# zyj0021200/simpleImageCaptionZoo

Measured on AMD Instinct MI355X. Metric: captions/sec (SCST step), BUTDDetection COCO14-size vocab, higher is better.
Workload: dtype f32

## Files before the change

### include/icz.h

```cpp
#ifndef ICZ_H_
#define ICZ_H_
#include <stddef.h>
#include <stdint.h>

#ifdef __cplusplus
extern "C" {
#endif

typedef enum {
    ICZ_OK = 0,
    ICZ_ERR_INVALID = -1,
    ICZ_ERR_HIP = -2,
    ICZ_ERR_STATE = -3,
    ICZ_ERR_NOMEM = -4
} icz_status;

const char* icz_last_error(void);
const char* icz_version(void);

typedef struct icz_butd icz_butd_t;

typedef struct {
    int32_t R;
    int32_t D;
// ... 268 lines not shown
                   const int32_t* img_ref_ptr, int32_t n_img, int32_t* stats_out, void* stream);
int icz_rouge_lcs(const int32_t* hyp_tok, const int32_t* hyp_ptr, const int32_t* ref_tok, const int32_t* ref_ptr,
                  const int32_t* img_ref_ptr, int32_t n_img, int32_t* lcs_out, void* stream);

int icz_gemm_f32(int32_t layout, const float* X, int32_t ldx, const float* W, int32_t ldw, const float* bias,
                 float* C, int32_t ldc, int32_t M, int32_t N, int32_t K, int32_t nsplit, float* workspace,
                 size_t workspace_floats, void* stream);
size_t icz_gemm_workspace_floats(int32_t M, int32_t N);
int icz_gemm_f32_seg(int32_t layout, int32_t nseg, const float* const* A, const int32_t* lda, const float* const* B, const int32_t* ldb,
                     const int32_t* K, const float* bias, float* C, int32_t ldc, int32_t M, int32_t N, int32_t nsplit, int32_t accumulate,
                     const int32_t* live, float* workspace, size_t workspace_floats, int32_t* nsplit_used, void* stream);
int icz_gemm_resident_pair(int32_t nseg_a, const float* const* A_a, const int32_t* lda_a, const float* const* B_a, const int32_t* ldb_a, const int32_t* K_a,
                           int32_t M_a, int32_t N_a, float* slabs_a, size_t slabs_a_floats, int32_t* nsplit_a,
                           int32_t nseg_b, const float* const* A_b, const int32_t* lda_b, const float* const* B_b, const int32_t* ldb_b, const int32_t* K_b,
                           int32_t M_b, int32_t N_b, float* slabs_b, size_t slabs_b_floats, int32_t* nsplit_b, const int32_t* live, void* stream);
int icz_gemm_set_big_cfg(int32_t cfg);
int icz_gemm_big_cfg_for(int32_t layout, int32_t M, int32_t N, int32_t K, int32_t nsplit);
int icz_gemm_tn_grouped(const float* dY, int32_t ldy, int32_t M, int32_t K, int32_t ngroups, const float* const* X, const int32_t* ldx,
                        const int32_t* cols, float* const* out, const int32_t* ldo, const int32_t* rows_live, void* stream);
int icz_gemm_tn_split_pick(int32_t M, int32_t N, int32_t K);
int icz_gemm_tn_split(const float* dY, int32_t ldy, int32_t M, const float* X, int32_t ldx, int32_t N, int32_t K, float* out, int32_t ldo,
                      float* workspace, size_t workspace_floats, const int32_t* rows_live, void* stream);
int icz_gemm_route_for(int32_t layout, int32_t M, int32_t N, int32_t nseg, const int32_t* K, int32_t nsplit);
int icz_gemm_split_for(int32_t layout, int32_t M, int32_t N, int32_t nseg, const int32_t* K, size_t workspace_floats);
int icz_gemm_tn_grouped_fits(int32_t M, int32_t K, int32_t ngroups, const int32_t* cols);
int icz_prof_begin(void);
int icz_prof_select(int32_t which);
int icz_prof_pair_overhead(void* stream, int32_t n, double* avg_us);
int icz_prof_end(double* avg_us, double* bytes_per_launch, double* flops_per_launch, long long* launches);
int icz_kprof_begin(void);
// ... 8 lines not shown
```

### simpleimagecaptionzoo_amd/_lib.py

```python
import ctypes as C
import os

_HERE = os.path.dirname(os.path.abspath(__file__))
LIB_PATH = os.path.join(_HERE, "libicz.so")


class IczError(RuntimeError):
    pass


GRAD_READY_CB = C.CFUNCTYPE(None, C.c_void_p, C.c_int32)


class ButdDims(C.Structure):
    _fields_ = [(n, C.c_int32) for n in ("R", "D", "H", "E", "A", "V", "max_rows", "max_len")]


BUTD_PARAM_FIELDS = (
    "embed_weight",
    "td_w_ih", "td_w_hh", "td_b_ih", "td_b_hh",
    "lm_w_ih", "lm_w_hh", "lm_b_ih", "lm_b_hh",
    "enc_att_v", "enc_att_g", "enc_att_b",
    "dec_att_v", "dec_att_g", "dec_att_b",
    "affine_v", "affine_g", "affine_b",
# ... 188 lines not shown
        "icz_ciderd_scores_csr": (C.c_int, [vp, vp, vp, i32, i32, vp, vp, vp, vp, vp, vp, vp, vp, vp, vp]),
        "icz_ngram_diversity": (C.c_int, [vp, vp, i32, i32, vp, vp]),
        "icz_bleu_stats": (C.c_int, [vp, vp, vp, vp, vp, i32, vp, vp]),
        "icz_rouge_lcs": (C.c_int, [vp, vp, vp, vp, vp, i32, vp, vp]),
        "icz_prof_begin": (C.c_int, []),
        "icz_prof_select": (C.c_int, [i32]),
        "icz_prof_pair_overhead": (C.c_int, [vp, i32, C.POINTER(C.c_double)]),
        "icz_prof_end": (C.c_int, [C.POINTER(C.c_double), C.POINTER(C.c_double), C.POINTER(C.c_double), C.POINTER(C.c_longlong)]),
        "icz_kprof_begin": (C.c_int, []),
        "icz_kprof_end": (C.c_int, [i32, C.POINTER(C.c_double), C.POINTER(C.c_longlong)]),
        "icz_prof_stream_rate": (C.c_int, [vp, C.c_size_t, i32, vp, C.POINTER(C.c_double)]),
        "icz_adam_clamp_multi": (C.c_int, [i32, C.POINTER(vp), C.POINTER(vp), C.POINTER(vp), C.POINTER(vp), C.POINTER(i64), f32, f32, i32, vp]),
        "icz_gemm_f32": (C.c_int, [i32, vp, i32, vp, i32, vp, vp, i32, i32, i32, i32, i32, vp, C.c_size_t, vp]),
        "icz_gemm_f32_seg": (C.c_int, [i32, i32, vp, vp, vp, vp, vp, vp, vp, i32, i32, i32, i32, i32, vp, vp, C.c_size_t, C.POINTER(i32), vp]),
        "icz_gemm_resident_pair": (C.c_int, [i32, vp, vp, vp, vp, vp, i32, i32, vp, C.c_size_t, C.POINTER(i32)] * 2 + [vp, vp]),
        "icz_gemm_workspace_floats": (C.c_size_t, [i32, i32]),
        "icz_gemm_set_big_cfg": (C.c_int, [i32]),
        "icz_gemm_big_cfg_for": (C.c_int, [i32, i32, i32, i32, i32]),
        "icz_gemm_tn_grouped": (C.c_int, [vp, i32, i32, i32, i32, vp, vp, vp, vp, vp, vp, vp]),
        "icz_gemm_tn_split_pick": (C.c_int, [i32, i32, i32]),
        "icz_gemm_tn_split": (C.c_int, [vp, i32, i32, vp, i32, i32, i32, vp, i32, vp, C.c_size_t, vp, vp]),
        "icz_gemm_route_for": (C.c_int, [i32, i32, i32, i32, vp, i32]),
        "icz_gemm_split_for": (C.c_int, [i32, i32, i32, i32, vp, C.c_size_t]),
        "icz_gemm_tn_grouped_fits": (C.c_int, [i32, i32, i32, vp]),
    }
    for name, (res, args) in sig.items():
        try:
            fn = getattr(L, name)
        except AttributeError as e:
            raise IczError("libicz.so lacks symbol %s (stale build?)" % name) from e
# ... 18 lines not shown
```

### simpleimagecaptionzoo_amd/butd.py

```python
import ctypes as C

import torch

from . import _lib
from ._lib import BUTD_PARAM_KEYS, ButdDims, ButdParams, Rng, check, lib, ptr, stream_ptr
from .handle import GraphDecoderHandle


def make_rng(seed=0, uniforms=None, emb_mask=None, att_mask=None, out_mask=None):
    r = Rng()
    r.seed = int(seed) & 0xFFFFFFFFFFFFFFFF
    keep = []
    for name, t, dt in (("uniforms", uniforms, torch.float32), ("emb_mask", emb_mask, torch.uint8),
                        ("att_mask", att_mask, torch.uint8), ("out_mask", out_mask, torch.uint8)):
        if t is not None:
            if t.dtype != dt or not t.is_cuda or not t.is_contiguous():
                raise _lib.IczError("%s must be a contiguous %s CUDA tensor" % (name, dt))
            setattr(r, name, t.data_ptr())
            keep.append(t)
    r._keep = keep
    return r


class ButdHandle(GraphDecoderHandle):
# ... 121 lines not shown
        M, N = (int(out.shape[0]), int(out.shape[1])) if out is not None else (1, 1)
    dev = out.device if out is not None else (As[0].device if n else "cuda")
    if out is None and not raw_slabs:
        out = torch.empty(M, N, device=dev, dtype=torch.float32)
    if workspace is None:
        workspace = torch.empty(max(lib().icz_gemm_workspace_floats(M, N), max(nsplit, 1) * M * N), device=dev, dtype=torch.float32)
    used = C.c_int32(0)
    c = None if raw_slabs else out
    check(lib().icz_gemm_f32_seg(code, n, ap, lda, bp, ldb, kk, ptr(bias), ptr(c), c.stride(0) if c is not None else N, M, N, int(nsplit),
                                 1 if accumulate else 0, ptr(live), ptr(workspace), workspace.numel(), C.byref(used), stream_ptr()))
    if info is not None:
        info["nsplit"] = used.value
    return workspace[:used.value * M * N].view(used.value, M, N) if raw_slabs else out


def gemm_resident_pair(As_a, Bs_a, As_b, Bs_b, slabs_a=None, slabs_b=None, live=None):
    ta, tb = _seg_tables("nt", As_a, Bs_a), _seg_tables("nt", As_b, Bs_b)
    bufs = []
    for (n, _, _, _, _, kk, M, N), buf, As in ((ta, slabs_a, As_a), (tb, slabs_b, As_b)):
        if M is None:
            raise _lib.IczError("gemm_resident_pair: a problem without segments")
        if buf is None:
            buf = torch.empty(max(sum(kk) // 256, 1) * M * N, device=As[0].device, dtype=torch.float32)
        bufs.append(buf)
    na, nb = C.c_int32(0), C.c_int32(0)
    args = []
    for (n, ap, lda, bp, ldb, kk, M, N), buf, used in ((ta, bufs[0], na), (tb, bufs[1], nb)):
        args += [n, ap, lda, bp, ldb, kk, M, N, ptr(buf), buf.numel(), C.byref(used)]
    check(lib().icz_gemm_resident_pair(*args, ptr(live), stream_ptr()))
    return tuple(buf[:u.value * t[6] * t[7]].view(u.value, t[6], t[7]) for t, buf, u in ((ta, bufs[0], na), (tb, bufs[1], nb)))


def gemm_set_big_cfg(cfg):
    check(lib().icz_gemm_set_big_cfg(int(cfg)))


def gemm_tn_grouped(dY, Xs, outs=None, rows_live=None):
    K, M = dY.shape
    n = len(Xs)
    if outs is None:
        outs = [torch.empty(M, x.shape[1], device=dY.device, dtype=torch.float32) for x in Xs]
    xp = (C.c_void_p * n)(*[x.data_ptr() for x in Xs])
    op = (C.c_void_p * n)(*[o.data_ptr() for o in outs])
    ldx = (C.c_int32 * n)(*[x.stride(0) for x in Xs])
# ... 44 lines not shown
```

### simpleimagecaptionzoo_amd/csrc/butd.hip

```cpp
#include <vector>

#include "butd_impl.h"

namespace icz {

int Butd::init(const icz_butd_dims& d) {
    dims = d;
    ICZ_REQUIRE(d.R > 0 && d.R <= 64, "butd: R=%d must be in 1..64 (36 boxes / 49 grid cells)", d.R);
    ICZ_REQUIRE(d.D % 4 == 0 && d.H % 4 == 0 && d.E % 4 == 0 && d.A % 4 == 0, "butd: D,H,E,A must be multiples of 4");
    ICZ_REQUIRE(d.V > 3 && d.max_rows > 0 && d.max_len > 0, "butd: bad V/max_rows/max_len");
    const size_t rows = d.max_rows, H = d.H, D = d.D, E = d.E, A = d.A, V = d.V, R = d.R;
    ICZ_TRY(alloc((void**)&w_enc, sizeof(float) * A * D));
    ICZ_TRY(alloc((void**)&w_dec, sizeof(float) * A * H));
    ICZ_TRY(alloc((void**)&w_aff, sizeof(float) * A));
    const size_t Vp = pad_vocab(d.V);
    ICZ_TRY(alloc((void**)&w_pred, sizeof(float) * Vp * H));
    ICZ_TRY(alloc((void**)&n_enc, sizeof(float) * A));
    ICZ_TRY(alloc((void**)&n_dec, sizeof(float) * A));
    ICZ_TRY(alloc((void**)&n_aff, sizeof(float) * 4));
    ICZ_TRY(alloc((void**)&n_pred, sizeof(float) * V));
    ICZ_TRY(alloc((void**)&mean, sizeof(float) * rows * D));
    ICZ_TRY(alloc((void**)&premean, sizeof(float) * rows * 4 * H));
    ICZ_TRY(alloc((void**)&enc_ctx, sizeof(float) * rows * R * A));
    for (int i = 0; i < 2; ++i) {
// ... 13 lines not shown
    ICZ_TRY(alloc((void**)&it, sizeof(int64_t) * rows));
    ICZ_TRY(alloc_scalars(mem));
    size_t nmax = 4 * H;
    if (A > nmax) nmax = A;
    if (V > nmax) nmax = V;
    ws_floats = (size_t)TARGET_WGS * 4096 * 2 + rows * nmax;
    {
        const size_t kmax = 2 * H + (E > D ? E : D), r128 = rows < 128 ? rows : 128;
        const size_t need = (kmax / 256 + 1) * r128 * 4 * H;
        if (need > ws_floats) ws_floats = need;
    }
    ICZ_TRY(alloc((void**)&ws, sizeof(float) * ws_floats));
    ICZ_TRY(mem.synced());
    if (const char* e = getenv("ICZ_EARLY_OUT")) early_out = atoi(e) != 0;
    if (const char* e = getenv("ICZ_MERGE_SMALL")) { const int n = atoi(e); if (n >= 0 && n <= 32) merge_small = n; }
    return ICZ_OK;
}

int Butd::refresh(hipStream_t st) {
    ICZ_REQUIRE(bound, "butd: parameters not bound");
    const int A = dims.A, D = dims.D, H = dims.H, V = dims.V;
    WeightNormTable wt = {};
    int nb = 0;
    auto add = [&](const float* v, const float* g, float* w, float* norm, int rows, int cols) {
        wt.j[wt.count++] = {v, g, w, norm, rows, cols, nb};
        nb += cdiv(rows, 4);
    };
    add(P.enc_att_v, P.enc_att_g, w_enc, n_enc, A, D);
    add(P.dec_att_v, P.dec_att_g, w_dec, n_dec, A, H);
    add(P.affine_v, P.affine_g, w_aff, n_aff, 1, A);
// ... 214 lines not shown
    }
    b->P = *p;
    b->bound = true;
    b->fresh = false;
    return ICZ_OK;
}

int icz_butd_set_option(icz_butd_t* h, const char* name, int32_t value) {
    ICZ_REQUIRE(h && name, "icz_butd_set_option: null argument");
    Butd* b = reinterpret_cast<Butd*>(h);
    if (strcmp(name, "graphs") == 0) { b->use_graphs = value != 0; return ICZ_OK; }
    if (strcmp(name, "concurrent") == 0) { b->concurrent = value != 0; return ICZ_OK; }
    if (strcmp(name, "early_out") == 0) { b->early_out = value != 0; return ICZ_OK; }
    if (strcmp(name, "small_nt") == 0) { b->small_nt = value != 0; return ICZ_OK; }
    if (strcmp(name, "group_att") == 0) { b->group_att = value != 0; return ICZ_OK; }
    if (strcmp(name, "merge_small") == 0) {
        ICZ_REQUIRE(value >= 0 && value <= 32, "icz_butd_set_option: merge_small %d outside 0..32", value);
        b->merge_small = value;
        return ICZ_OK;
    }
    set_error("icz_butd_set_option: unknown option '%s'", name);
    return ICZ_ERR_INVALID;
}

int icz_butd_set_mask_sum_global(icz_butd_t* h, const float* mask_sum_global_dev, void* stream) {
    return set_norm_global("icz_butd_set_mask_sum_global", reinterpret_cast<Butd*>(h), mask_sum_global_dev, stream);
}

int icz_butd_set_grad_callback(icz_butd_t* h, icz_grad_ready_cb cb, void* user) {
    ICZ_REQUIRE(h, "null handle");
// ... 39 lines not shown
```

### simpleimagecaptionzoo_amd/csrc/butd_impl.h

```cpp
#pragma once
#include <vector>
#include <stdint.h>

#include "decoder_core.h"

namespace icz {

struct StepIO {
    int rows;
    const float* feats;
    const int32_t* img_of_row;
    int rows_per_img;
    const int64_t* it;
    bool emb_ready;
    const float *h1_in, *c1_in, *h2_in, *c2_in;
    float *h1_out, *c1_out, *h2_out, *c2_out;
    float* emb_out;
    float* gates_td_out;
    float* gates_lm_out;
    float* dec_ctx_out;
    float* alpha_out;
    float* alpha_out2; int alpha2_stride;
    float* ctx_out;
    float* h2drop_out;
// ... 48 lines not shown
    int refresh_transposes(hipStream_t st);

    int alloc(void** p, size_t bytes) { return mem.alloc(p, bytes); }
    int init(const icz_butd_dims& d);
    int refresh(hipStream_t st);
    int gemm_nt(GemmArgs& g, const float* bias, hipStream_t st);
    int prologue(const float* feats, int n_img, hipStream_t st);
    int step(const StepIO& s, hipStream_t st);
    int zero_state(int rows, int which, hipStream_t st);
    int greedy(const float* feats, int B, int max_len, int64_t* ids_out, float* alphas_out, hipStream_t st);

    GraphCache gc{24};
    bool use_graphs = false;
    bool concurrent = true;
    uintptr_t opt_bits() const {
        return (concurrent ? 1 : 0) + (early_out ? 2 : 0) + 4 * merge_small + (small_nt ? 256 : 0) + (group_att ? 512 : 0);
    }
    int greedy_impl(const float* feats, int B, int max_len, int64_t* ids_out, float* alphas_out, hipStream_t st);
    int sample_impl(const float* feats, int B, int T, int64_t* seq_out, float* logp_out, hipStream_t st);
    int greedy_chain(const float* feats, int B, int max_len, int64_t* ids_out, float* alphas_out, hipStream_t st, bool scst = false);
    int sample_chain(const float* feats, int B, int T, int64_t* seq_out, float* logp_out, hipStream_t st, int row0 = 0, int64_t* ids_out = nullptr);
    int rollouts(const float* feats, int B, int T, const icz_rng* r, int64_t* ids_out, int64_t* seq_out, float* logp_out, hipStream_t st);
    int rollouts_impl(const float* feats, int B, int T, int64_t* ids_out, int64_t* seq_out, float* logp_out, hipStream_t st);
    SideStream side;
    SideStream low;
    icz_grad_ready_cb grad_cb = nullptr; void* grad_cb_user = nullptr;
    int sample_backward_impl(const float* reward, const icz_butd_params& G, float* loss_out, float* mask_sum_out, hipStream_t st,
                             int phases = 0xF, bool fire_cb = true);
    bool bptt_joined = false;
    int merge_small = 8;
    int cur_rows = 0, cur_row0 = 0;
    bool early_out = true;
    bool bptt_early_out = false;
    bool small_nt = true;
    int cur_K = 1, cur_nimg = 0;
    bool group_att = false;

    const float* seam_feats = nullptr;
    int vocab() const override { return dims.V; }
    int row_capacity() const override { return dims.max_rows; }
    bool refreshed() const override { return fresh; }
    bool compact_step() const override { return true; }
    EmbSlot emb_slot() const override { return {P.embed_weight, emb, dims.E, 1}; }
    DeviceBuffers& buffers() override { return mem; }
    int prologue(const float* feats, int n_img, int k, const int32_t* img_of_row, hipStream_t st) override;
    int step(int rows, const int64_t* it, const int32_t* img_of_row, int rows_per_img, int cur, bool slabs, LogitsView* out,
             hipStream_t st) override;
    void gather(const int32_t* src_row, int rows, int fan, hipStream_t st) override;

// ... 26 lines not shown
```

### simpleimagecaptionzoo_amd/csrc/butd_train.hip

```cpp
#include <math.h>

#include "butd_impl.h"

namespace icz {

__global__ void sample_init_kernel(uint8_t* unf, int* nunf, int64_t* tok, int B, int T) {
    const int i = blockIdx.x * blockDim.x + threadIdx.x;
    if (i < B) { unf[i] = 1; tok[i] = 1; }
    if (i < T) nunf[i] = 0;
}

int Butd::ensure_train(int B, int T) {
    if (tb.B >= B && tb.T >= T) return ICZ_OK;
    ICZ_REQUIRE(B <= 2 * dims.max_rows, "butd: batch %d exceeds capacity %d", B, dims.max_rows);
    ICZ_REQUIRE(T <= XE_MAX_T, "butd: %d steps exceed the limit of %d", T, XE_MAX_T);
    if (tb.B > B) B = tb.B;
    if (tb.T > T) T = tb.T;
    if (dims.max_len > T) T = dims.max_len;
    if (!mem.training.empty()) {
        ICZ_TRY(mem.release_training(&gc));
        tb = TrainBuf();
        drop_loss_buffers();
    }
    if (!wt_lm_ih && wt_possible()) {
// ... 446 lines not shown
        }
        const bool rdg = wt_lm_ih && wt_fresh && bt > 32 && bt <= 64 && gemm_slab_floats(bt, D + H, 4 * H / 256) <= tb.xfloats &&
                         gemm_slab_floats(bt, H, 2 * (4 * H / 256)) <= tb.xfloats;
        const bool tdg = small_nt && wt_lm_ih && wt_fresh && bt <= 32;
        const GemmLayout lay = (rdg || tdg) ? GEMM_NT : GEMM_NN;
        const float* const dglm = tb.dGlm + slot * 4 * H;
        const float* const dgtd = tb.dGtd + slot * 4 * H;
        auto wseg = [&](const float* dg, const float* w_t, const float* w, int ldw) -> GemmSeg {
            return lay == GEMM_NT ? GemmSeg{dg, w_t, 4 * H, 4 * H, 4 * H} : GemmSeg{dg, w, 4 * H, ldw, 4 * H};
        };
        auto dgrad = [&](GemmArgs g, float* slab, int* ns) -> int {
            if (!rdg) return gemm_auto(lay, g, slab, tb.xfloats, ns, st);
            *ns = gemm_resident_x3_nsplit(g);
            return gemm_slabs(GEMM_NT, g, *ns, slab, tb.xfloats, st, "butd");
        };
        ICZ_TRY(dgrad(gemm_args({wseg(dglm, wt_lm_ih, P.lm_w_ih, D + H)}, bt, D + H, tb.X[0], D + H, live), tb.X[0], &ns1));
        {
            const int dparts = cdiv(D, DALPHA_COLS);
            hipLaunchKernelGGL(att_bwd_dalpha_kernel, dim3(bt, dparts), dim3(256), 0, st, tb.X[0], ns1, D + H, bt, feats, R, D, tb.dalpha, live, imgk);
            AttBwdDdecArgs da = {enc_ctx, tb.dec + slot * A, w_aff, tb.alpha + slot * R, tb.dalpha, tb.dDec + slot * A, tb.dS + slot * R, R, A, dparts, live, imgk};
            hipLaunchKernelGGL(att_bwd_ddec_kernel, dim3(bt, cdiv(A, 256)), dim3(256), 0, st, da, d_att);
            GemmArgs g = gemm_args({{tb.dDec + slot * A, w_dec, A, H, A}}, bt, H, tb.X[1], H, live);
            ICZ_TRY(gemm_auto(GEMM_NN, g, tb.X[1], tb.xfloats, &ns2, st));
        }
        {
            LstmBwdArgs a = {};
            a.dh_a = bnext ? tb.X[3] : nullptr; a.ns_a = ns4; a.lda_a = H; a.rows_a = bnext;
            a.dh_b = tb.X[0] + D; a.ns_b = ns1; a.lda_b = D + H; a.rows_b = bt;
            a.dh_c = tb.X[1]; a.ns_c = ns2; a.lda_c = H; a.rows_c = bt;
            a.dc_in = bnext ? tb.dc1[cur] : nullptr; a.dc_in_rows = bnext;
            a.gates = tb.gtd + slot * 4 * H;
            a.c_prev = tb.c1 + slot * H; a.c_cur = tb.c1 + slot * H + sH;
            a.dgates = tb.dGtd + slot * 4 * H; a.dc_prev = tb.dc1[cur ^ 1];
            a.rows = bt; a.H = H; a.live = live; a.carry_live = carry_live;
            hipLaunchKernelGGL(lstm_bwd_point_kernel, dim3(cdiv(H, 256), bt), dim3(256), 0, st, a, d_off);
        }
        if (t > 0) {
            const GemmArgs g3 = gemm_args({wseg(dglm, wt_lm_hh, P.lm_w_hh, H), wseg(dgtd, wt_td_ih_h2, P.td_w_ih, H + D + E)}, bt, H, tb.X[2], H, live);
            const GemmArgs g4 = gemm_args({wseg(dgtd, wt_td_hh, P.td_w_hh, H)}, bt, H, tb.X[3], H, live);
            if (rdg) {
                ns3 = gemm_resident_x3_nsplit(g3); ns4 = gemm_resident_x3_nsplit(g4);
                ICZ_REQUIRE(gemm_slab_floats(bt, H, ns3) <= tb.xfloats, "butd: slab buffer too small for the dgrad slabs");
                ICZ_TRY(gemm_resident_x3_pair(g3, g4, st));
            } else {
                ICZ_TRY(dgrad(g3, tb.X[2], &ns3));
                ICZ_TRY(dgrad(g4, tb.X[3], &ns4));
            }
        }
        bnext = bt;
        cur ^= 1;
    }
    return ICZ_OK;
    };
    const int s_loop = loop();
    if (grad_cb || s_loop != ICZ_OK) {
// ... 214 lines not shown
```

### simpleimagecaptionzoo_amd/csrc/gemm_f32.h

```cpp
#pragma once
#include "icz_common.h"

namespace icz {

constexpr int GEMM_MAX_SEG = 4;
constexpr int GEMM_BM = 64, GEMM_BN = 64, GEMM_BK = 64;

enum GemmLayout { GEMM_NT = 0, GEMM_NN = 1, GEMM_TN = 2 };

struct GemmSeg {
    const float* A;
    const float* B;
    int lda, ldb;
    int K;
    const int64_t* gather;
};

struct GemmArgs {
    GemmSeg seg[GEMM_MAX_SEG];
    int nseg;
    int M, N;
    float* out;
    int ldo;
    const float* bias;
// ... 2 lines not shown
    int accumulate;
    int spread;
    const int* live;
    const int* rows_live;
};

int gemm_f32(GemmLayout layout, const GemmArgs& a, hipStream_t stream);
int gemm_route(GemmLayout layout, const GemmArgs& a);
int gemm_pick_split(const GemmArgs& a, int target_wgs, GemmLayout layout = GEMM_NT);
int gemm_pick_split_balanced(const GemmArgs& a, GemmLayout layout, size_t slab_capacity_floats);
size_t gemm_slab_floats(int M, int N, int nsplit);
int gemm_normalize_split(GemmLayout layout, const GemmArgs& a, int nsplit);
int gemm_fit_split(GemmLayout layout, const GemmArgs& a, int nsplit, size_t capacity_floats);

bool gemm_resident_x3_fits(const GemmArgs& a);
int gemm_resident_x3_stages(const GemmArgs& a);
int gemm_resident_x3_nsplit(const GemmArgs& a);
int gemm_resident_x3(const GemmArgs& a, hipStream_t stream);
bool gemm_resident_x3_pair_fits(const GemmArgs& a, const GemmArgs& b);
int gemm_resident_x3_pair(const GemmArgs& a, const GemmArgs& b, hipStream_t stream);
int gemm_predict(const float* x, int H, const float* w_pred, const float* bias, int rows, int V, int Vp, float* logits, int ldl,
                 float* ws, size_t ws_cap_floats, int* pred_nsplit, hipStream_t st, const int* live = nullptr);

int gemm_big_x3(GemmLayout layout, const GemmArgs& a, int cfg, hipStream_t stream);
int gemm_big_cfg(GemmLayout layout, const GemmArgs& a);
int gemm_big_switch();
void gemm_set_big_cfg(int cfg);
constexpr int GEMM_MAX_COLGROUPS = 4;
struct GemmColGroup { const float* B; int ldb; int cols; float* out; int ldo; };
bool gemm_tn_grouped_fits(int M, int K, const GemmColGroup* groups, int ngroups);
int gemm_tn_grouped(const float* dY, int ldy, int M, int K, const GemmColGroup* groups, int ngroups, const int* rows_live, hipStream_t stream);

int gemm_tn_split_pick(int M, int N, int K);
int gemm_tn_split(const float* dY, int ldy, int M, const float* X, int ldx, int N, int K, int nsplit, float* slabs, const int* rows_live, hipStream_t st);
struct GemmSwitches { bool tn_x3, nn_x3, nt_x3big, resident_x3, resident_m128, predict_slabs, resident_k512; unsigned prof_every; int big_cfg; };
// ... 4 lines not shown
```

### simpleimagecaptionzoo_amd/csrc/gemm_f32.hip

```cpp
#include <stdlib.h>

#include <array>
#include <mutex>
#include <set>
#include <vector>

#include "gemm_ops.h"

namespace icz {

static int total_chunks(const GemmArgs& a, int bk = GEMM_BK) {
    int t = 0;
    for (int s = 0; s < a.nseg; ++s) t += cdiv(a.seg[s].K, bk);
    return t;
}

template <int BK>
struct ChunkCursorT {
    int seg, k0;
    const float* A; const float* B;
    int lda, ldb, K;
    __device__ __forceinline__ void load_seg(const GemmArgs& a) {
        const GemmSeg& g = a.seg[seg];
        A = g.A; B = g.B; lda = g.lda; ldb = g.ldb; K = g.K;
// ... 1259 lines not shown
    if (C) {
        g.out = C; g.ldo = ldc;
        ICZ_TRY(gemm_finished(lay, g, ns, bias, workspace, workspace_floats, st, "icz_gemm_f32_seg"));
    } else {
        g.out = workspace; g.ldo = N; g.bias = bias; g.nsplit = ns;
        ICZ_TRY(gemm_f32(lay, g, st));
    }
    if (nsplit_used) *nsplit_used = ns;
    return ICZ_OK;
}

int icz_gemm_resident_pair(int32_t nseg_a, const float* const* A_a, const int32_t* lda_a, const float* const* B_a, const int32_t* ldb_a, const int32_t* K_a,
                           int32_t M_a, int32_t N_a, float* slabs_a, size_t slabs_a_floats, int32_t* nsplit_a,
                           int32_t nseg_b, const float* const* A_b, const int32_t* lda_b, const float* const* B_b, const int32_t* ldb_b, const int32_t* K_b,
                           int32_t M_b, int32_t N_b, float* slabs_b, size_t slabs_b_floats, int32_t* nsplit_b, const int32_t* live, void* stream) {
    GemmArgs ga, gb;
    ICZ_TRY(seg_args("icz_gemm_resident_pair (first)", nseg_a, A_a, lda_a, B_a, ldb_a, K_a, M_a, N_a, &ga));
    ICZ_TRY(seg_args("icz_gemm_resident_pair (second)", nseg_b, A_b, lda_b, B_b, ldb_b, K_b, M_b, N_b, &gb));
    ga.out = slabs_a; ga.ldo = N_a; ga.live = live;
    gb.out = slabs_b; gb.ldo = N_b; gb.live = live;
    ICZ_REQUIRE(gemm_resident_x3_pair_fits(ga, gb), "icz_gemm_resident_pair: the two problems do not share a stage form of the resident kernel");
    ga.nsplit = gemm_resident_x3_nsplit(ga);
    gb.nsplit = gemm_resident_x3_nsplit(gb);
    ICZ_REQUIRE(ga.nsplit > 1 && gb.nsplit > 1, "icz_gemm_resident_pair: slab products only (one k range: %d, %d)", ga.nsplit, gb.nsplit);
    ICZ_TRY(check_args(GEMM_NT, ga));
    ICZ_TRY(check_args(GEMM_NT, gb));
    ICZ_REQUIRE(((uintptr_t)slabs_a & 15) == 0 && ((uintptr_t)slabs_b & 15) == 0, "icz_gemm_resident_pair: slabs must be 16-byte aligned");
    ICZ_REQUIRE(gemm_slab_floats(M_a, N_a, ga.nsplit) <= slabs_a_floats && gemm_slab_floats(M_b, N_b, gb.nsplit) <= slabs_b_floats,
                "icz_gemm_resident_pair: slab buffers too small (%d x %d x %d, %d x %d x %d)", ga.nsplit, M_a, N_a, gb.nsplit, M_b, N_b);
    ICZ_TRY(gemm_resident_x3_pair(ga, gb, (hipStream_t)stream));
    if (nsplit_a) *nsplit_a = ga.nsplit;
    if (nsplit_b) *nsplit_b = gb.nsplit;
    return ICZ_OK;
}

int icz_gemm_set_big_cfg(int32_t cfg) {
    ICZ_REQUIRE(cfg >= -2 && cfg <= 5, "icz_gemm_set_big_cfg: %d", cfg);
    gemm_set_big_cfg(cfg);
    return ICZ_OK;
}

int icz_gemm_big_cfg_for(int32_t layout, int32_t M, int32_t N, int32_t K, int32_t nsplit) {
    if (layout < 0 || layout > 2 || M <= 0 || N <= 0 || K <= 0) return -1;
    GemmArgs g = {};
    g.nseg = 1;
// ... 64 lines not shown
```

### simpleimagecaptionzoo_amd/csrc/gemm_resident_x3.hip

```cpp
#include <stdlib.h>

#include <type_traits>

#include "gemm_f32.h"

namespace icz {

template <int I, int N, class F>
__device__ __forceinline__ void sk_static_for(F&& f) {
    if constexpr (I < N) {
        f(std::integral_constant<int, I>{});
        sk_static_for<I + 1, N>(f);
    }
}

typedef __attribute__((ext_vector_type(8))) __bf16 sk_bf16x8;
typedef __attribute__((ext_vector_type(4))) uint32_t sk_u32x4;
typedef __attribute__((ext_vector_type(2))) uint32_t sk_u32x2;

__device__ __forceinline__ uint32_t sk_cvt_pk_bf16(float lo, float hi) {
    uint32_t r;
    asm("v_cvt_pk_bf16_f32 %0, %1, %2" : "=v"(r) : "v"(lo), "v"(hi));
    return r;
}
// ... 489 lines not shown
    });
    stamp(31);
}

template <int D, bool STAMPS = false>
__global__ __launch_bounds__(256) void gemm_resident_x3_m128_kernel(GemmArgs a) {
    resident_x3_m128_body<D, STAMPS>(a, blockIdx.x);
}
constexpr size_t rs_m128_lds_bytes() { return (size_t)3 * 128 * rs_pb(2) * 2; }

static int rs_total_stages(const GemmArgs& a) {
    int tot = 0;
    for (int s = 0; s < a.nseg; ++s) tot += a.seg[s].K / SK_BK;
    return tot;
}
int gemm_resident_x3_stages(const GemmArgs& a) {
    const int tot = rs_total_stages(a);
    if (gemm_switches().resident_k512 && a.M <= 64 && tot % 8 == 0) return 8;
    return tot % 4 == 0 ? 4 : 0;
}
static bool rs_shape_ok(const GemmArgs& a) {
    if (!gemm_switches().resident_x3 || a.M <= 32 || a.M > (gemm_switches().resident_m128 ? 128 : 64) || a.N % 4 || a.accumulate) return false;
    for (int s = 0; s < a.nseg; ++s)
        if (a.seg[s].K % SK_BK || a.seg[s].gather) return false;
    return rs_total_stages(a) >= 8 && gemm_resident_x3_stages(a) > 0;
}
bool gemm_resident_x3_fits(const GemmArgs& a) { return a.N >= 2048 && rs_shape_ok(a); }
int gemm_resident_x3_nsplit(const GemmArgs& a) { return rs_total_stages(a) / gemm_resident_x3_stages(a); }

template <int NSR, bool STAMPS>
static int rs_launch(const GemmArgs& a, hipStream_t stream) {
    constexpr size_t lds = rs_lds_bytes<4, NSR>();
    static bool attr = false;
    if (!attr) {
        ICZ_CHECK_HIP(hipFuncSetAttribute(reinterpret_cast<const void*>(gemm_resident_x3_kernel<4, NSR, 2, 3, STAMPS>), hipFuncAttributeMaxDynamicSharedMemorySize, (int)lds));
        attr = true;
    }
    hipLaunchKernelGGL((gemm_resident_x3_kernel<4, NSR, 2, 3, STAMPS>), dim3(cdiv(a.N, 256) * a.nsplit), dim3(256), lds, stream, a);
    ICZ_CHECK_HIP(hipGetLastError());
    return ICZ_OK;
}

#ifndef RS_K512_D
// ... 34 lines not shown
    GemmArgs a = a_in;
    const int nsr = gemm_resident_x3_stages(a);
    ICZ_REQUIRE(rs_shape_ok(a) && a.nsplit == gemm_resident_x3_nsplit(a) && a.chunks_per_split == nsr,
                "gemm_resident_x3: launch does not match the kernel's fixed decomposition (nsplit %d)", a.nsplit);
    ICZ_REQUIRE(a.nsplit > 1 || a.ldo >= a.N, "gemm_resident_x3: output row stride %d below N = %d", a.ldo, a.N);
#ifdef ICZ_DEV
    if (rs_dev_env("ICZ_DEV_STAMPS")) {
        if (!g_sk_stamps) ICZ_CHECK_HIP(hipMalloc((void**)&g_sk_stamps, sizeof(unsigned long long) * 32 * 4096));
        a.bias = reinterpret_cast<const float*>(g_sk_stamps);
        return a.M > 64 ? rs_launch_m128<true>(a, stream) : (nsr == 8 ? rs_launch_k512<true>(a, stream) : rs_launch<4, true>(a, stream));
    }
#endif
    return a.M > 64 ? rs_launch_m128<false>(a, stream) : (nsr == 8 ? rs_launch_k512<false>(a, stream) : rs_launch<4, false>(a, stream));
}

bool gemm_resident_x3_pair_fits(const GemmArgs& a, const GemmArgs& b) {
    return a.M <= 64 && b.M <= 64 && rs_shape_ok(a) && rs_shape_ok(b) && gemm_resident_x3_stages(a) == gemm_resident_x3_stages(b) && a.N >= 512 && b.N >= 512;
}
int gemm_resident_x3_pair(const GemmArgs& a_in, const GemmArgs& b_in, hipStream_t stream) {
    ICZ_REQUIRE(gemm_resident_x3_pair_fits(a_in, b_in), "gemm_resident_x3_pair: shapes outside the kernel's decomposition");
    GemmPair g;
    g.a = a_in; g.b = b_in;
    const int nsr = gemm_resident_x3_stages(g.a), tilew = nsr == 8 ? 128 : 256;
    for (GemmArgs* p : {&g.a, &g.b}) {
        p->nsplit = gemm_resident_x3_nsplit(*p);
        p->chunks_per_split = nsr;
        p->bias = nullptr;
        ICZ_REQUIRE(p->out && p->nsplit > 1, "gemm_resident_x3_pair: slab output expected");
    }
    g.first = cdiv(g.a.N, tilew) * g.a.nsplit;
    constexpr size_t lds = rs_lds_bytes<4, 4>();
    static bool attr = false;
    if (!attr) {
        ICZ_CHECK_HIP(hipFuncSetAttribute(reinterpret_cast<const void*>(gemm_resident_x3_pair_kernel<4, 4, 2, 3>), hipFuncAttributeMaxDynamicSharedMemorySize, (int)lds));
        ICZ_CHECK_HIP(hipFuncSetAttribute(reinterpret_cast<const void*>(gemm_resident_x3_pair_kernel<4, 8, 1, RS_K512_D, 4>), hipFuncAttributeMaxDynamicSharedMemorySize, (int)lds));
        attr = true;
    }
    const dim3 grid(g.first + cdiv(g.b.N, tilew) * g.b.nsplit);
    if (nsr == 8) hipLaunchKernelGGL((gemm_resident_x3_pair_kernel<4, 8, 1, RS_K512_D, 4>), grid, dim3(256), lds, stream, g);
    else hipLaunchKernelGGL((gemm_resident_x3_pair_kernel<4, 4, 2, 3>), grid, dim3(256), lds, stream, g);
    ICZ_CHECK_HIP(hipGetLastError());
    return ICZ_OK;
}

int gemm_predict(const float* x, int H, const float* w_pred, const float* bias, int rows, int V, int Vp, float* logits, int ldl,
                 float* ws, size_t ws_cap_floats, int* pred_nsplit, hipStream_t st, const int* live) {
    GemmArgs g = {};
    g.nseg = 1;
    g.live = live;
    g.seg[0] = {x, w_pred, H, H, H, nullptr};
    g.M = rows; g.N = Vp; g.out = ws; g.ldo = Vp;
    if (gemm_switches().predict_slabs && pred_nsplit && ws && gemm_resident_x3_fits(g) && gemm_resident_x3_nsplit(g) > 1 &&
        gemm_slab_floats(rows, Vp, gemm_resident_x3_nsplit(g)) <= ws_cap_floats) {
        g.nsplit = gemm_resident_x3_nsplit(g);
// ... 18 lines not shown
```

Baseline: 11870.

## Regroup BPTT dgrad GEMMs by producer into paired resident launches

In the backward-through-time step, the dgrad GEMMs are regrouped by producer. The lm_ih dgrad is paired with the lm_hh part of the former fused g3, and the td_ih part is paired with td_hh in a second paired launch. This lets the lm-derived products start earlier and balances the work across the two launches. It also adds a 4-stage, 128-wide tile variant of the paired resident kernel, selectable by stage count and made the default via dgrad_by_producer=2, which raises the split count and grid size for small M. The cost is more slab partials to reduce and a new kernel instantiation, and the path only runs when the slab buffers fit.

```diff
diff --git a/include/icz.h b/include/icz.h
--- a/include/icz.h
+++ b/include/icz.h
@@ -306,6 +306,11 @@
                            int32_t M_a, int32_t N_a, float* slabs_a, size_t slabs_a_floats, int32_t* nsplit_a,
                            int32_t nseg_b, const float* const* A_b, const int32_t* lda_b, const float* const* B_b, const int32_t* ldb_b, const int32_t* K_b,
                            int32_t M_b, int32_t N_b, float* slabs_b, size_t slabs_b_floats, int32_t* nsplit_b, const int32_t* live, void* stream);
+int icz_gemm_resident_pair_stages(int32_t nseg_a, const float* const* A_a, const int32_t* lda_a, const float* const* B_a, const int32_t* ldb_a, const int32_t* K_a,
+                                  int32_t M_a, int32_t N_a, float* slabs_a, size_t slabs_a_floats, int32_t* nsplit_a,
+                                  int32_t nseg_b, const float* const* A_b, const int32_t* lda_b, const float* const* B_b, const int32_t* ldb_b, const int32_t* K_b,
+                                  int32_t M_b, int32_t N_b, float* slabs_b, size_t slabs_b_floats, int32_t* nsplit_b, int32_t stages,
+                                  const int32_t* live, void* stream);
 int icz_gemm_set_big_cfg(int32_t cfg);
 int icz_gemm_big_cfg_for(int32_t layout, int32_t M, int32_t N, int32_t K, int32_t nsplit);
 int icz_gemm_tn_grouped(const float* dY, int32_t ldy, int32_t M, int32_t K, int32_t ngroups, const float* const* X, const int32_t* ldx,
diff --git a/simpleimagecaptionzoo_amd/_lib.py b/simpleimagecaptionzoo_amd/_lib.py
--- a/simpleimagecaptionzoo_amd/_lib.py
+++ b/simpleimagecaptionzoo_amd/_lib.py
@@ -226,6 +226,7 @@
         "icz_gemm_f32": (C.c_int, [i32, vp, i32, vp, i32, vp, vp, i32, i32, i32, i32, i32, vp, C.c_size_t, vp]),
         "icz_gemm_f32_seg": (C.c_int, [i32, i32, vp, vp, vp, vp, vp, vp, vp, i32, i32, i32, i32, i32, vp, vp, C.c_size_t, C.POINTER(i32), vp]),
         "icz_gemm_resident_pair": (C.c_int, [i32, vp, vp, vp, vp, vp, i32, i32, vp, C.c_size_t, C.POINTER(i32)] * 2 + [vp, vp]),
+        "icz_gemm_resident_pair_stages": (C.c_int, [i32, vp, vp, vp, vp, vp, i32, i32, vp, C.c_size_t, C.POINTER(i32)] * 2 + [i32, vp, vp]),
         "icz_gemm_workspace_floats": (C.c_size_t, [i32, i32]),
         "icz_gemm_set_big_cfg": (C.c_int, [i32]),
         "icz_gemm_big_cfg_for": (C.c_int, [i32, i32, i32, i32, i32]),
diff --git a/simpleimagecaptionzoo_amd/butd.py b/simpleimagecaptionzoo_amd/butd.py
--- a/simpleimagecaptionzoo_amd/butd.py
+++ b/simpleimagecaptionzoo_amd/butd.py
@@ -159,7 +159,7 @@
     return workspace[:used.value * M * N].view(used.value, M, N) if raw_slabs else out
 
 
-def gemm_resident_pair(As_a, Bs_a, As_b, Bs_b, slabs_a=None, slabs_b=None, live=None):
+def gemm_resident_pair(As_a, Bs_a, As_b, Bs_b, slabs_a=None, slabs_b=None, live=None, stages=0):
     ta, tb = _seg_tables("nt", As_a, Bs_a), _seg_tables("nt", As_b, Bs_b)
     bufs = []
     for (n, _, _, _, _, kk, M, N), buf, As in ((ta, slabs_a, As_a), (tb, slabs_b, As_b)):
@@ -172,7 +172,10 @@
     args = []
     for (n, ap, lda, bp, ldb, kk, M, N), buf, used in ((ta, bufs[0], na), (tb, bufs[1], nb)):
         args += [n, ap, lda, bp, ldb, kk, M, N, ptr(buf), buf.numel(), C.byref(used)]
-    check(lib().icz_gemm_resident_pair(*args, ptr(live), stream_ptr()))
+    if stages:
+        check(lib().icz_gemm_resident_pair_stages(*args, int(stages), ptr(live), stream_ptr()))
+    else:
+        check(lib().icz_gemm_resident_pair(*args, ptr(live), stream_ptr()))
     return tuple(buf[:u.value * t[6] * t[7]].view(u.value, t[6], t[7]) for t, buf, u in ((ta, bufs[0], na), (tb, bufs[1], nb)))
 
 
diff --git a/simpleimagecaptionzoo_amd/csrc/butd.hip b/simpleimagecaptionzoo_amd/csrc/butd.hip
--- a/simpleimagecaptionzoo_amd/csrc/butd.hip
+++ b/simpleimagecaptionzoo_amd/csrc/butd.hip
@@ -51,6 +51,7 @@
     ICZ_TRY(mem.synced());
     if (const char* e = getenv("ICZ_EARLY_OUT")) early_out = atoi(e) != 0;
     if (const char* e = getenv("ICZ_MERGE_SMALL")) { const int n = atoi(e); if (n >= 0 && n <= 32) merge_small = n; }
+    if (const char* e = getenv("ICZ_DGRAD_BY_PRODUCER")) { const int n = atoi(e); if (n >= 0 && n <= 2) dgrad_by_producer = n; }
     return ICZ_OK;
 }
 
@@ -295,6 +296,11 @@
     if (strcmp(name, "early_out") == 0) { b->early_out = value != 0; return ICZ_OK; }
     if (strcmp(name, "small_nt") == 0) { b->small_nt = value != 0; return ICZ_OK; }
     if (strcmp(name, "group_att") == 0) { b->group_att = value != 0; return ICZ_OK; }
+    if (strcmp(name, "dgrad_by_producer") == 0) {
+        ICZ_REQUIRE(value >= 0 && value <= 2, "icz_butd_set_option: dgrad_by_producer %d outside 0..2", value);
+        b->dgrad_by_producer = value;
+        return ICZ_OK;
+    }
     if (strcmp(name, "merge_small") == 0) {
         ICZ_REQUIRE(value >= 0 && value <= 32, "icz_butd_set_option: merge_small %d outside 0..32", value);
         b->merge_small = value;
diff --git a/simpleimagecaptionzoo_amd/csrc/butd_impl.h b/simpleimagecaptionzoo_amd/csrc/butd_impl.h
--- a/simpleimagecaptionzoo_amd/csrc/butd_impl.h
+++ b/simpleimagecaptionzoo_amd/csrc/butd_impl.h
@@ -86,7 +86,7 @@
     bool use_graphs = false;
     bool concurrent = true;
     uintptr_t opt_bits() const {
-        return (concurrent ? 1 : 0) + (early_out ? 2 : 0) + 4 * merge_small + (small_nt ? 256 : 0) + (group_att ? 512 : 0);
+        return (concurrent ? 1 : 0) + (early_out ? 2 : 0) + 4 * merge_small + (small_nt ? 256 : 0) + (group_att ? 512 : 0) + 1024 * dgrad_by_producer;
     }
     int greedy_impl(const float* feats, int B, int max_len, int64_t* ids_out, float* alphas_out, hipStream_t st);
     int sample_impl(const float* feats, int B, int T, int64_t* seq_out, float* logp_out, hipStream_t st);
@@ -105,6 +105,7 @@
     bool early_out = true;
     bool bptt_early_out = false;
     bool small_nt = true;
+    int dgrad_by_producer = 2;
     int cur_K = 1, cur_nimg = 0;
     bool group_att = false;
 
diff --git a/simpleimagecaptionzoo_amd/csrc/butd_train.hip b/simpleimagecaptionzoo_amd/csrc/butd_train.hip
--- a/simpleimagecaptionzoo_amd/csrc/butd_train.hip
+++ b/simpleimagecaptionzoo_amd/csrc/butd_train.hip
@@ -484,7 +484,26 @@
             *ns = gemm_resident_x3_nsplit(g);
             return gemm_slabs(GEMM_NT, g, *ns, slab, tb.xfloats, st, "butd");
         };
-        ICZ_TRY(dgrad(gemm_args({wseg(dglm, wt_lm_ih, P.lm_w_ih, D + H)}, bt, D + H, tb.X[0], D + H, live), tb.X[0], &ns1));
+        const int stb = dgrad_by_producer == 2 ? 4 : 0;
+        const GemmArgs g1 = gemm_args({wseg(dglm, wt_lm_ih, P.lm_w_ih, D + H)}, bt, D + H, tb.X[0], D + H, live);
+        GemmArgs g3a = gemm_args({wseg(dglm, wt_lm_hh, P.lm_w_hh, H)}, bt, H, tb.X[2], H, live);
+        GemmArgs g3b = gemm_args({wseg(dgtd, wt_td_ih_h2, P.td_w_ih, H + D + E)}, bt, H, tb.X[2], H, live);
+        int ns3a = 0, ns3b = 0, ns4b = 0;
+        bool byp = rdg && t > 0 && dgrad_by_producer > 0;
+        if (byp) {
+            const GemmArgs g4 = gemm_args({wseg(dgtd, wt_td_hh, P.td_w_hh, H)}, bt, H, tb.X[3], H, live);
+            byp = gemm_resident_x3_pair_fits(g1, g3a) && gemm_resident_x3_pair_fits(g3b, g4, stb);
+            if (byp) {
+                ns3a = gemm_resident_x3_nsplit(g3a); ns3b = gemm_resident_x3_nsplit(g3b, stb); ns4b = gemm_resident_x3_nsplit(g4, stb);
+                byp = ns3a > 1 && ns3b > 1 && ns4b > 1 && gemm_slab_floats(bt, D + H, gemm_resident_x3_nsplit(g1)) <= tb.xfloats &&
+                      gemm_slab_floats(bt, H, ns3a + ns3b) <= tb.xfloats && gemm_slab_floats(bt, H, ns4b) <= tb.xfloats;
+            }
+        }
+        if (byp) {
+            ns1 = gemm_resident_x3_nsplit(g1);
+            ICZ_TRY(gemm_resident_x3_pair(g1, g3a, st));
+        } else
+            ICZ_TRY(dgrad(g1, tb.X[0], &ns1));
         {
             const int dparts = cdiv(D, DALPHA_COLS);
             hipLaunchKernelGGL(att_bwd_dalpha_kernel, dim3(bt, dparts), dim3(256), 0, st, tb.X[0], ns1, D + H, bt, feats, R, D, tb.dalpha, live, imgk);
@@ -508,7 +527,11 @@
         if (t > 0) {
             const GemmArgs g3 = gemm_args({wseg(dglm, wt_lm_hh, P.lm_w_hh, H), wseg(dgtd, wt_td_ih_h2, P.td_w_ih, H + D + E)}, bt, H, tb.X[2], H, live);
             const GemmArgs g4 = gemm_args({wseg(dgtd, wt_td_hh, P.td_w_hh, H)}, bt, H, tb.X[3], H, live);
-            if (rdg) {
+            if (byp) {
+                g3b.out = tb.X[2] + gemm_slab_floats(bt, H, ns3a);
+                ns3 = ns3a + ns3b; ns4 = ns4b;
+                ICZ_TRY(gemm_resident_x3_pair(g3b, g4, st, stb));
+            } else if (rdg) {
                 ns3 = gemm_resident_x3_nsplit(g3); ns4 = gemm_resident_x3_nsplit(g4);
                 ICZ_REQUIRE(gemm_slab_floats(bt, H, ns3) <= tb.xfloats, "butd: slab buffer too small for the dgrad slabs");
                 ICZ_TRY(gemm_resident_x3_pair(g3, g4, st));
diff --git a/simpleimagecaptionzoo_amd/csrc/gemm_f32.h b/simpleimagecaptionzoo_amd/csrc/gemm_f32.h
--- a/simpleimagecaptionzoo_amd/csrc/gemm_f32.h
+++ b/simpleimagecaptionzoo_amd/csrc/gemm_f32.h
@@ -40,11 +40,11 @@
 int gemm_fit_split(GemmLayout layout, const GemmArgs& a, int nsplit, size_t capacity_floats);
 
 bool gemm_resident_x3_fits(const GemmArgs& a);
-int gemm_resident_x3_stages(const GemmArgs& a);
-int gemm_resident_x3_nsplit(const GemmArgs& a);
+int gemm_resident_x3_stages(const GemmArgs& a, int stages = 0);
+int gemm_resident_x3_nsplit(const GemmArgs& a, int stages = 0);
 int gemm_resident_x3(const GemmArgs& a, hipStream_t stream);
-bool gemm_resident_x3_pair_fits(const GemmArgs& a, const GemmArgs& b);
-int gemm_resident_x3_pair(const GemmArgs& a, const GemmArgs& b, hipStream_t stream);
+bool gemm_resident_x3_pair_fits(const GemmArgs& a, const GemmArgs& b, int stages = 0);
+int gemm_resident_x3_pair(const GemmArgs& a, const GemmArgs& b, hipStream_t stream, int stages = 0);
 int gemm_predict(const float* x, int H, const float* w_pred, const float* bias, int rows, int V, int Vp, float* logits, int ldl,
                  float* ws, size_t ws_cap_floats, int* pred_nsplit, hipStream_t st, const int* live = nullptr);
 
diff --git a/simpleimagecaptionzoo_amd/csrc/gemm_f32.hip b/simpleimagecaptionzoo_amd/csrc/gemm_f32.hip
--- a/simpleimagecaptionzoo_amd/csrc/gemm_f32.hip
+++ b/simpleimagecaptionzoo_amd/csrc/gemm_f32.hip
@@ -1297,21 +1297,31 @@
                            int32_t M_a, int32_t N_a, float* slabs_a, size_t slabs_a_floats, int32_t* nsplit_a,
                            int32_t nseg_b, const float* const* A_b, const int32_t* lda_b, const float* const* B_b, const int32_t* ldb_b, const int32_t* K_b,
                            int32_t M_b, int32_t N_b, float* slabs_b, size_t slabs_b_floats, int32_t* nsplit_b, const int32_t* live, void* stream) {
+    return icz_gemm_resident_pair_stages(nseg_a, A_a, lda_a, B_a, ldb_a, K_a, M_a, N_a, slabs_a, slabs_a_floats, nsplit_a,
+                                         nseg_b, A_b, lda_b, B_b, ldb_b, K_b, M_b, N_b, slabs_b, slabs_b_floats, nsplit_b, 0, live, stream);
+}
+
+int icz_gemm_resident_pair_stages(int32_t nseg_a, const float* const* A_a, const int32_t* lda_a, const float* const* B_a, const int32_t* ldb_a, const int32_t* K_a,
+                                  int32_t M_a, int32_t N_a, float* slabs_a, size_t slabs_a_floats, int32_t* nsplit_a,
+                                  int32_t nseg_b, const float* const* A_b, const int32_t* lda_b, const float* const* B_b, const int32_t* ldb_b, const int32_t* K_b,
+                                  int32_t M_b, int32_t N_b, float* slabs_b, size_t slabs_b_floats, int32_t* nsplit_b, int32_t stages,
+                                  const int32_t* live, void* stream) {
+    ICZ_REQUIRE(stages == 0 || stages == 4 || stages == 8, "icz_gemm_resident_pair: %d stages per k range is no form of the resident kernel (0, 4, 8)", stages);
     GemmArgs ga, gb;
     ICZ_TRY(seg_args("icz_gemm_resident_pair (first)", nseg_a, A_a, lda_a, B_a, ldb_a, K_a, M_a, N_a, &ga));
     ICZ_TRY(seg_args("icz_gemm_resident_pair (second)", nseg_b, A_b, lda_b, B_b, ldb_b, K_b, M_b, N_b, &gb));
     ga.out = slabs_a; ga.ldo = N_a; ga.live = live;
     gb.out = slabs_b; gb.ldo = N_b; gb.live = live;
-    ICZ_REQUIRE(gemm_resident_x3_pair_fits(ga, gb), "icz_gemm_resident_pair: the two problems do not share a stage form of the resident kernel");
-    ga.nsplit = gemm_resident_x3_nsplit(ga);
-    gb.nsplit = gemm_resident_x3_nsplit(gb);
+    ICZ_REQUIRE(gemm_resident_x3_pair_fits(ga, gb, stages), "icz_gemm_resident_pair: the two problems do not share a stage form of the resident kernel");
+    ga.nsplit = gemm_resident_x3_nsplit(ga, stages);
+    gb.nsplit = gemm_resident_x3_nsplit(gb, stages);
     ICZ_REQUIRE(ga.nsplit > 1 && gb.nsplit > 1, "icz_gemm_resident_pair: slab products only (one k range: %d, %d)", ga.nsplit, gb.nsplit);
     ICZ_TRY(check_args(GEMM_NT, ga));
     ICZ_TRY(check_args(GEMM_NT, gb));
     ICZ_REQUIRE(((uintptr_t)slabs_a & 15) == 0 && ((uintptr_t)slabs_b & 15) == 0, "icz_gemm_resident_pair: slabs must be 16-byte aligned");
     ICZ_REQUIRE(gemm_slab_floats(M_a, N_a, ga.nsplit) <= slabs_a_floats && gemm_slab_floats(M_b, N_b, gb.nsplit) <= slabs_b_floats,
                 "icz_gemm_resident_pair: slab buffers too small (%d x %d x %d, %d x %d x %d)", ga.nsplit, M_a, N_a, gb.nsplit, M_b, N_b);
-    ICZ_TRY(gemm_resident_x3_pair(ga, gb, (hipStream_t)stream));
+    ICZ_TRY(gemm_resident_x3_pair(ga, gb, (hipStream_t)stream, stages));
     if (nsplit_a) *nsplit_a = ga.nsplit;
     if (nsplit_b) *nsplit_b = gb.nsplit;
     return ICZ_OK;
diff --git a/simpleimagecaptionzoo_amd/csrc/gemm_resident_x3.hip b/simpleimagecaptionzoo_amd/csrc/gemm_resident_x3.hip
--- a/simpleimagecaptionzoo_amd/csrc/gemm_resident_x3.hip
+++ b/simpleimagecaptionzoo_amd/csrc/gemm_resident_x3.hip
@@ -527,10 +527,12 @@
     for (int s = 0; s < a.nseg; ++s) tot += a.seg[s].K / SK_BK;
     return tot;
 }
-int gemm_resident_x3_stages(const GemmArgs& a) {
+int gemm_resident_x3_stages(const GemmArgs& a, int stages) {
     const int tot = rs_total_stages(a);
-    if (gemm_switches().resident_k512 && a.M <= 64 && tot % 8 == 0) return 8;
-    return tot % 4 == 0 ? 4 : 0;
+    const int own = (gemm_switches().resident_k512 && a.M <= 64 && tot % 8 == 0) ? 8 : (tot % 4 == 0 ? 4 : 0);
+    if (stages == 0) return own;
+    if (stages == 4) return a.M <= 64 && tot % 4 == 0 ? 4 : 0;
+    return stages == 8 && own == 8 ? 8 : 0;
 }
 static bool rs_shape_ok(const GemmArgs& a) {
     if (!gemm_switches().resident_x3 || a.M <= 32 || a.M > (gemm_switches().resident_m128 ? 128 : 64) || a.N % 4 || a.accumulate) return false;
@@ -539,7 +541,10 @@
     return rs_total_stages(a) >= 8 && gemm_resident_x3_stages(a) > 0;
 }
 bool gemm_resident_x3_fits(const GemmArgs& a) { return a.N >= 2048 && rs_shape_ok(a); }
-int gemm_resident_x3_nsplit(const GemmArgs& a) { return rs_total_stages(a) / gemm_resident_x3_stages(a); }
+int gemm_resident_x3_nsplit(const GemmArgs& a, int stages) {
+    const int nsr = gemm_resident_x3_stages(a, stages);
+    return nsr ? rs_total_stages(a) / nsr : 0;
+}
 
 template <int NSR, bool STAMPS>
 static int rs_launch(const GemmArgs& a, hipStream_t stream) {
@@ -604,16 +609,17 @@
     return a.M > 64 ? rs_launch_m128<false>(a, stream) : (nsr == 8 ? rs_launch_k512<false>(a, stream) : rs_launch<4, false>(a, stream));
 }
 
-bool gemm_resident_x3_pair_fits(const GemmArgs& a, const GemmArgs& b) {
-    return a.M <= 64 && b.M <= 64 && rs_shape_ok(a) && rs_shape_ok(b) && gemm_resident_x3_stages(a) == gemm_resident_x3_stages(b) && a.N >= 512 && b.N >= 512;
-}
-int gemm_resident_x3_pair(const GemmArgs& a_in, const GemmArgs& b_in, hipStream_t stream) {
-    ICZ_REQUIRE(gemm_resident_x3_pair_fits(a_in, b_in), "gemm_resident_x3_pair: shapes outside the kernel's decomposition");
+bool gemm_resident_x3_pair_fits(const GemmArgs& a, const GemmArgs& b, int stages) {
+    const int sa = gemm_resident_x3_stages(a, stages), sb = gemm_resident_x3_stages(b, stages);
+    return a.M <= 64 && b.M <= 64 && rs_shape_ok(a) && rs_shape_ok(b) && sa > 0 && sa == sb && a.N >= 512 && b.N >= 512;
+}
+int gemm_resident_x3_pair(const GemmArgs& a_in, const GemmArgs& b_in, hipStream_t stream, int stages) {
+    ICZ_REQUIRE(gemm_resident_x3_pair_fits(a_in, b_in, stages), "gemm_resident_x3_pair: shapes outside the kernel's decomposition (stages %d)", stages);
     GemmPair g;
     g.a = a_in; g.b = b_in;
-    const int nsr = gemm_resident_x3_stages(g.a), tilew = nsr == 8 ? 128 : 256;
+    const int nsr = gemm_resident_x3_stages(g.a, stages), tilew = (nsr == 8 || stages == 4) ? 128 : 256;
     for (GemmArgs* p : {&g.a, &g.b}) {
-        p->nsplit = gemm_resident_x3_nsplit(*p);
+        p->nsplit = gemm_resident_x3_nsplit(*p, stages);
         p->chunks_per_split = nsr;
         p->bias = nullptr;
         ICZ_REQUIRE(p->out && p->nsplit > 1, "gemm_resident_x3_pair: slab output expected");
@@ -623,11 +629,13 @@
     static bool attr = false;
     if (!attr) {
         ICZ_CHECK_HIP(hipFuncSetAttribute(reinterpret_cast<const void*>(gemm_resident_x3_pair_kernel<4, 4, 2, 3>), hipFuncAttributeMaxDynamicSharedMemorySize, (int)lds));
+        ICZ_CHECK_HIP(hipFuncSetAttribute(reinterpret_cast<const void*>(gemm_resident_x3_pair_kernel<4, 4, 1, 3>), hipFuncAttributeMaxDynamicSharedMemorySize, (int)lds));
         ICZ_CHECK_HIP(hipFuncSetAttribute(reinterpret_cast<const void*>(gemm_resident_x3_pair_kernel<4, 8, 1, RS_K512_D, 4>), hipFuncAttributeMaxDynamicSharedMemorySize, (int)lds));
         attr = true;
     }
     const dim3 grid(g.first + cdiv(g.b.N, tilew) * g.b.nsplit);
     if (nsr == 8) hipLaunchKernelGGL((gemm_resident_x3_pair_kernel<4, 8, 1, RS_K512_D, 4>), grid, dim3(256), lds, stream, g);
+    else if (stages == 4) hipLaunchKernelGGL((gemm_resident_x3_pair_kernel<4, 4, 1, 3>), grid, dim3(256), lds, stream, g);
     else hipLaunchKernelGGL((gemm_resident_x3_pair_kernel<4, 4, 2, 3>), grid, dim3(256), lds, stream, g);
     ICZ_CHECK_HIP(hipGetLastError());
     return ICZ_OK;
```

After: 11950, median of 6. About the same (+0.6%).
